# ipc-sim/IPC

Measured on AMD Instinct MI355X. Metric: newton_iterations_per_sec, higher is better.
Workload: dtype f64

## Files before the change

### ipc_amd/csrc/mf_numeric.hip

```cpp
#include <climits>
#include "mf_kernels.h"
#include "device_prims.h"
#include <algorithm>
#include <chrono>
#include <cstdio>
#include <cstdlib>
#include <cstring>
#include <thread>

namespace ipcgpu {

namespace {

__global__ void k_clear_flag(int* __restrict__ flag) { flag[0] = 0; }


struct EntryView {
    const int *ia, *ja;
    int nRows, ns;
    const int *newOf, *nodeFront, *firstNode, *idxPtr, *idx;
    const long long* frontOff;
    const int4* frontInfo;
};
__global__ __launch_bounds__(256) void k_entry_dst(EntryView v, long long* __restrict__ dst, int* __restrict__ bucket, int* __restrict__ hist)
{
    const int r = blockIdx.x * 4 + (threadIdx.x >> 6), lane = threadIdx.x & 63;
    if (r >= v.nRows) return;
    const int pr = 3 * v.newOf[r / 3] + r % 3;
    for (int k = v.ia[r] + lane; k < v.ia[r + 1]; k += 64) {
        const int c = v.ja[k];
        const int pc = 3 * v.newOf[c / 3] + c % 3;
        const int i = max(pr, pc), j = min(pr, pc);
        const int s = v.nodeFront[j / 3];
        const int f = v.firstNode[s], l = v.firstNode[s + 1];
        const int nIdx = v.idxPtr[s + 1] - v.idxPtr[s];
        int lr;
        if (i / 3 < l) lr = i - 3 * f;
        else {
            const int* b = v.idx + v.idxPtr[s] + (l - f);
            int lo = 0, hi = nIdx - (l - f);
            const int key = i / 3;
            while (lo < hi) {
                const int mid = (lo + hi) >> 1;
                if (b[mid] < key) lo = mid + 1;
                else hi = mid;
            }
            lr = 3 * ((l - f) + lo) + i % 3;
        }
        const int lc = j - 3 * f;
        dst[k] = v.frontOff[s] + lr + (long long)(3 * nIdx) * lc;
        const int4 info = v.frontInfo[s];
        int bkt = -1;
        if (info.x == 0) bkt = s;
        else if (info.x > 0) {
            const int ti = lr / TS, tj = lc / TS, cT = info.z;
            bkt = v.ns + info.y + (ti <= cT ? ti * (ti + 1) / 2 : cT * (cT + 1) / 2 + (ti - cT) * cT) + tj;
        }
        bucket[k] = bkt;
        if (bkt >= 0) atomicAdd(&hist[bkt], 1);
    }
}
__global__ __launch_bounds__(1024) void k_scan_exclusive(int n, const int* __restrict__ in, int* __restrict__ out)
{
    __shared__ int part[1024];
    const int t = threadIdx.x;
    const int chunk = (n + 1023) / 1024;
    const int b = min(t * chunk, n), e = min(b + chunk, n);
    int sum = 0;
    for (int i = b; i < e; ++i) sum += in[i];
    part[t] = sum;
    __syncthreads();
    for (int off = 1; off < 1024; off <<= 1) {
        const int x = (t >= off) ? part[t - off] : 0;
        __syncthreads();
        part[t] += x;
        __syncthreads();
    }
    int run = part[t] - sum;
    for (int i = b; i < e; ++i) {
        out[i] = run;
        run += in[i];
    }
    if (t == 1023) out[n] = part[1023];
}
__global__ void k_entry_scatter(int nnz, int ns, const long long* __restrict__ dst, const int* __restrict__ bucket, const int* __restrict__ start,
    int* __restrict__ cursor, const long long* __restrict__ frontOff, int2* __restrict__ aEnt, int* __restrict__ bigSrc,
    long long* __restrict__ bigDst)
{
    const int k = blockIdx.x * blockDim.x + threadIdx.x;
    if (k >= nnz) return;
    const int b = bucket[k];
    if (b < 0) return;
    const int pos = start[b] + atomicAdd(&cursor[b], 1);
    if (b < ns) {
        aEnt[pos] = make_int2((int)(dst[k] - frontOff[b]), k);
    }
    else {
        const int q = pos - start[ns];
        bigSrc[q] = k;
        bigDst[q] = dst[k];
    }
}

#ifdef MF_EA_PROBE
constexpr int EA_PROBE_PH = 8;
__device__ unsigned long long g_eaProbe[2][64][EA_PROBE_PH + 1];
struct EaProbe {
    unsigned long long t[EA_PROBE_PH];
};
#define EA_PROBE_DECL EaProbe pr_ = {}
#define EA_STAMP(k)                                                                                                                                           \
    do {                                                                                                                                                      \
        if (probeLevel >= 0) {                                                                                                                                \
            asm volatile("s_waitcnt vmcnt(0) lgkmcnt(0)" ::: "memory");                                                                                       \
            if (threadIdx.x == 0) pr_.t[k] = wall_clock64();                                                                                                  \
        }                                                                                                                                                     \
    } while (0)
__device__ inline void ea_probe_flush(const EaProbe& p, int kernel, int level)
{
    if (threadIdx.x != 0 || level < 0 || level >= 64) return;
    unsigned long long prev = p.t[0];
    for (int k = 1; k < EA_PROBE_PH; ++k) {
        const unsigned long long t = p.t[k] ? p.t[k] : prev;
        atomicAdd(&g_eaProbe[kernel][level][k], t - prev);
        prev = t;
    }
    atomicAdd(&g_eaProbe[kernel][level][EA_PROBE_PH], 1ull);
}
#define EA_PROBE_FLUSH(kernel) ea_probe_flush(pr_, kernel, probeLevel)
#else
#define EA_PROBE_DECL do {} while (0)
#define EA_STAMP(k) do {} while (0)
#define EA_PROBE_FLUSH(kernel) do {} while (0)
#endif

struct KidGather {
    double x[16];
    bool ok[16];
};
__device__ __forceinline__ void kid_gather(const double* __restrict__ Fc, const long long Nc, const int r, const int (&cc)[16], KidGather& g)
{
#pragma unroll
    for (int q = 0; q < 16; ++q) {
        g.ok[q] = r >= 0 && cc[q] >= 0 && r >= cc[q];
        g.x[q] = Fc[g.ok[q] ? r + Nc * cc[q] : 0];
    }
}
__device__ __forceinline__ const double* kid_front(const double* fronts, const int4 k)
{
    return fronts + (((long long)(unsigned)k.y << 32) | (unsigned)k.x);
}

__global__ __launch_bounds__(WG) void k_extend_add(const int4* __restrict__ tile, const int* __restrict__ childMap, const int4* __restrict__ kidRec,
    double* __restrict__ fronts, int ownOnly, const int* __restrict__ aPtr, const int* __restrict__ aSrc, const long long* __restrict__ aDst,
    const double* __restrict__ a
#ifdef MF_EA_PROBE
    ,
    int probeLevel
#endif
)
{
    EA_PROBE_DECL;
    EA_STAMP(0);
    const int4 g = tile[4 * blockIdx.x], t = tile[4 * blockIdx.x + 1], k0 = tile[4 * blockIdx.x + 2], k1 = tile[4 * blockIdx.x + 3];
    const int aBeg = aPtr[blockIdx.x], aEnd = aPtr[blockIdx.x + 1];
    const int tid = threadIdx.x, lane = tid & 63, wv = __builtin_amdgcn_readfirstlane(tid >> 6);
    const int e0 = aBeg + tid;
    long long dst0 = 0;
    double a0 = 0.0;
    if (e0 < aEnd) {
        dst0 = aDst[e0];
        a0 = a[aSrc[e0]];
    }
    EA_STAMP(1);
    const int N = g.x, ncOwn = g.y, nk = t.z;
    double* F = fronts + (((long long)(unsigned)g.w << 32) | (unsigned)g.z);
    const int I = TS * t.x + lane, J0 = TS * t.y + 16 * wv;
    const int* m0 = childMap + k0.w;
    const int* m1 = childMap + k1.w;
    const int r0 = m0[I], r1 = m1[I];
    int c0[16], c1[16];
#pragma unroll
    for (int q = 0; q < 16; ++q) {
        c0[q] = m0[J0 + q];
        c1[q] = m1[J0 + q];
    }
    EA_STAMP(2);
    KidGather g0, g1;
    kid_gather(kid_front(fronts, k0), k0.z, r0, c0, g0);
    kid_gather(kid_front(fronts, k1), k1.z, r1, c1, g1);
    double sum[16];
#pragma unroll
    for (int q = 0; q < 16; ++q) sum[q] = 0.0;
#pragma unroll
    for (int q = 0; q < 16; ++q) sum[q] += g0.ok[q] ? g0.x[q] : 0.0;
#pragma unroll
    for (int q = 0; q < 16; ++q) sum[q] += g1.ok[q] ? g1.x[q] : 0.0;
    EA_STAMP(4);
    for (int k = 2; k < nk; ++k) {
        const int4 kr = kidRec[t.w + k];
        const int* m = childMap + kr.w;
        const int r = m[I];
#pragma unroll
        for (int q = 0; q < 16; ++q) c0[q] = m[J0 + q];
        kid_gather(kid_front(fronts, kr), kr.z, r, c0, g0);
#pragma unroll
        for (int q = 0; q < 16; ++q) sum[q] += g0.ok[q] ? g0.x[q] : 0.0;
    }
    if (I < N) {
#pragma unroll
        for (int q = 0; q < 16; ++q) {
            const int J = J0 + q;
            if (J <= I && (!ownOnly || J < ncOwn)) F[I + (long long)N * J] = sum[q];
        }
    }
    EA_STAMP(6);
    if (aBeg < aEnd) {
        __syncthreads();
        if (e0 < aEnd) fronts[dst0] += a0;
        for (int e = e0 + WG; e < aEnd; e += WG) fronts[aDst[e]] += a[aSrc[e]];
    }
    EA_STAMP(7);
    EA_PROBE_FLUSH(0);
}

__device__ __forceinline__ double bcast_lane(double v, int lane)
{
    const int lo = __builtin_amdgcn_readlane(__double2loint(v), lane);
    const int hi = __builtin_amdgcn_readlane(__double2hiint(v), lane);
    return __hiloint2double(hi, lo);
}

__device__ __forceinline__ double rsqrt_nr(double d)
{
    double r = __builtin_amdgcn_rsq(d);
    double e = fma(-d * r, r, 1.0);
    r = fma(0.5 * r, e, r);
    e = fma(-d * r, r, 1.0);
    r = fma(0.5 * r, e, r);
    return r;
}

__device__ __forceinline__ double rcp_nr(double d)
{
    double r = __builtin_amdgcn_rcp(d);
    double e = fma(-d, r, 1.0);
    r = fma(r, e, r);
    e = fma(-d, r, 1.0);
    r = fma(r, e, r);
    return r;
}

__device__ __forceinline__ double lane_xor16(double v) { return __shfl_xor(v, 16, 64); }

__device__ __forceinline__ bool wave_potrf_inv32_mfma(const double* blk, int ld, int w, int lane, double* Xs)
{
    const int lo = lane & 15, hi = lane >> 4;
    f64x4 T00, T01, T11, W00, W11;
    f64x4 W10 = { 0.0, 0.0, 0.0, 0.0 };
    f64x4 aV0, bV0, dV0, alV0, cbV0, aV1, bV1, dV1;
    const int wm = w - 1;
#pragma unroll
    for (int r = 0; r < 4; ++r) {
        const int q = hi + 4 * r;
        const int mn = min(q, lo), mx = max(q, lo);
        const double a00 = blk[min(mn, wm) * ld + min(mx, wm)];
        const double a01 = blk[min(q, wm) * ld + min(16 + lo, wm)];
        const double a11 = blk[min(16 + mn, wm) * ld + min(16 + mx, wm)];
        const bool dg = q == lo;
        T00[r] = (mx < w) ? a00 : (dg ? 1.0 : 0.0);
        T01[r] = (16 + lo < w) ? a01 : 0.0;
        T11[r] = (16 + mx < w) ? a11 : (dg ? 1.0 : 0.0);
        W00[r] = dg ? 1.0 : 0.0;
        W11[r] = dg ? 1.0 : 0.0;
        aV0[r] = aV1[r] = dV0[r] = dV1[r] = 1.0;
        bV0[r] = bV1[r] = alV0[r] = cbV0[r] = 0.0;
    }
    bool bad = false;
#pragma unroll
    for (int k = 0; k < 16; k += 2) {
        if (k >= w) break;
        const int h = k & 3, r = k >> 2;
        const bool selh = hi == h, both = (hi >> 1) == (h >> 1), live = both && lo > k + 1;
        const double row = T00[r];
        const double partner = lane_xor16(row);
        const double a = bcast_lane(row, 16 * h + k), b = bcast_lane(row, 16 * h + k + 1), c = bcast_lane(row, 16 * (h + 1) + k + 1);
        const double det = fma(a, c, -(b * b));
        bad |= !(a > 0.0) || !(det > 0.0);
        const double rdet = rcp_nr(det);
        const double ca = c * rdet, cb = b * rdet, cc = a * rdet;
        const double alpha = selh ? ca : cc;
        const double m = live ? fma(-alpha, row, cb * partner) : 0.0;
        T00 = __builtin_amdgcn_mfma_f64_16x16x4f64(m, row, T00, 0, 0, 0);
        T01 = __builtin_amdgcn_mfma_f64_16x16x4f64(m, T01[r], T01, 0, 0, 0);
        W00 = __builtin_amdgcn_mfma_f64_16x16x4f64(m, W00[r], W00, 0, 0, 0);
        aV0[r] = both ? a : aV0[r];
        bV0[r] = both ? b : bV0[r];
        dV0[r] = both ? det : dV0[r];
        alV0[r] = both ? alpha : alV0[r];
        cbV0[r] = both ? cb : cbV0[r];
    }
    if (w > 16) {
#pragma unroll
        for (int ks = 0; ks < 4; ++ks) {
            const double t = T01[ks];
            const double a = fma(-alV0[ks], t, cbV0[ks] * lane_xor16(t));
            T11 = __builtin_amdgcn_mfma_f64_16x16x4f64(a, t, T11, 0, 0, 0);
            W10 = __builtin_amdgcn_mfma_f64_16x16x4f64(a, W00[ks], W10, 0, 0, 0);
        }
#pragma unroll
        for (int k = 0; k < 16; k += 2) {
            if (16 + k >= w) break;
            const int h = k & 3, r = k >> 2;
            const bool selh = hi == h, both = (hi >> 1) == (h >> 1), live = both && lo > k + 1;
            const double row = T11[r];
            const double partner = lane_xor16(row);
            const double a = bcast_lane(row, 16 * h + k), b = bcast_lane(row, 16 * h + k + 1), c = bcast_lane(row, 16 * (h + 1) + k + 1);
            const double det = fma(a, c, -(b * b));
            bad |= !(a > 0.0) || !(det > 0.0);
            const double rdet = rcp_nr(det);
            const double ca = c * rdet, cb = b * rdet, cc = a * rdet;
            const double alpha = selh ? ca : cc;
            const double m = live ? fma(-alpha, row, cb * partner) : 0.0;
            T11 = __builtin_amdgcn_mfma_f64_16x16x4f64(m, row, T11, 0, 0, 0);
            W11 = __builtin_amdgcn_mfma_f64_16x16x4f64(m, W11[r], W11, 0, 0, 0);
            aV1[r] = both ? a : aV1[r];
            bV1[r] = both ? b : bV1[r];
            dV1[r] = both ? det : dV1[r];
        }
    }
    const bool even = (hi & 1) == 0;
#pragma unroll
    for (int r = 0; r < 4; ++r) {
        const int q = hi + 4 * r;
        const double ia0 = rsqrt_nr(aV0[r]), iv0 = ia0 * ia0, il0 = rsqrt_nr(dV0[r] * iv0);
        const double ia1 = rsqrt_nr(aV1[r]), iv1 = ia1 * ia1, il1 = rsqrt_nr(dV1[r] * iv1);
        const double p0 = even ? ia0 : il0, q0 = even ? 0.0 : -bV0[r] * iv0 * il0;
        const double p1 = even ? ia1 : il1, q1 = even ? 0.0 : -bV1[r] * iv1 * il1;
        const double w0 = W00[r], w1 = W11[r];
        Xs[lo * LDX + q] = fma(q0, lane_xor16(w0), p0 * w0);
        Xs[(16 + lo) * LDX + 16 + q] = fma(q1, lane_xor16(w1), p1 * w1);
        Xs[(16 + lo) * LDX + q] = 0.0;
    }
    __builtin_amdgcn_fence(__ATOMIC_SEQ_CST, "wavefront");
    __builtin_amdgcn_wave_barrier();
    f64x4 X10 = { 0.0, 0.0, 0.0, 0.0 };
    if (w > 16) {
#pragma unroll
        for (int ks = 0; ks < 4; ++ks)
            X10 = __builtin_amdgcn_mfma_f64_16x16x4f64(Xs[(16 + 4 * ks + hi) * LDX + 16 + lo], W10[ks], X10, 0, 0, 0);
    }
#pragma unroll
    for (int r = 0; r < 4; ++r) Xs[lo * LDX + 16 + hi + 4 * r] = X10[r];
    __builtin_amdgcn_fence(__ATOMIC_SEQ_CST, "wavefront");
    __builtin_amdgcn_wave_barrier();
    return bad;
}

#ifndef MF_FUSED_SCHUR_GROUP
#define MF_FUSED_SCHUR_GROUP 2
#endif
#ifdef MF_FUSED_PROBE
__device__ unsigned long long g_probe[16 << 16];
__device__ const int* g_probeBase;
#define MF_PROBE(slot) do { if (tid == 0) g_probe[16 * probeId + (slot)] = wall_clock64(); } while (0)
#define MF_PROBE_ACC(var) do { if (tid == 0) { const unsigned long long now_ = wall_clock64(); var += now_ - probeLast; probeLast = now_; } } while (0)
#else
#define MF_PROBE(slot) do {} while (0)
#define MF_PROBE_ACC(var) do {} while (0)
#endif
template <int NT>
__global__ __launch_bounds__(NT, 3) void k_front_fused(const int* __restrict__ fdesc, const int* __restrict__ invMap,
    const int2* __restrict__ aEnt, const double* __restrict__ a, double* __restrict__ fronts,
    double* __restrict__ dinv, int* __restrict__ flag, int* __restrict__ flagNext)
{
    extern __shared__ double P[];
    __shared__ double Xs[NB * LDX];
    __shared__ __attribute__((aligned(16))) int fd[FD_STRIDE];
    const int tid = threadIdx.x, lane = tid & 63, wv = tid >> 6;
    if (tid < FD_STRIDE) fd[tid] = fdesc[(size_t)blockIdx.x * FD_STRIDE + tid];
    if (flagNext && blockIdx.x == 0 && tid == 0) flagNext[0] = 0;
    __syncthreads();
    const int N = fd[2], nc = fd[3], nk = fd[8];
    double* F = fronts + *reinterpret_cast<const long long*>(fd);
    double* dblk = dinv + *reinterpret_cast<const long long*>(fd + 4) * (NB * NB);
    const int aBeg = fd[6], aEnd = fd[7];
    int* cm = reinterpret_cast<int*>(P + (size_t)nc * N);
    bool bad = false;
#ifdef MF_FUSED_PROBE
    const long long probeId = ((fdesc - g_probeBase) / FD_STRIDE + blockIdx.x) & 0xffff;
    unsigned long long probeLast = 0, probePivot = 0, probeRows = 0, probeTrail = 0, probeGather = 0, probeTiles = 0;
    if (tid == 0) {
        g_probe[16 * probeId + 12] = N;
        g_probe[16 * probeId + 13] = nc;
        g_probe[16 * probeId + 14] = nk;
    }
#endif
    MF_PROBE(0);
    const int aLast = max(aEnd - 1, 0);
    int2 ent0[4];
    double av0[4];
#pragma unroll
    for (int u = 0; u < 4; ++u) ent0[u] = aEnt[min(aBeg + u * NT + tid, aLast)];
    for (int q = 0; q < nk; ++q) {
        const int* inv = invMap + fd[16 + 6 * q + 4];
        const int ncc = fd[16 + 6 * q + 3];
        for (int I = tid; I < N; I += NT) {
            const int In = I / 3;
            const int ic = inv[In];
            cm[q * N + I] = ic >= 0 ? ncc + 3 * ic + (I - 3 * In) : -1;
        }
    }
#pragma unroll
    for (int u = 0; u < 4; ++u) av0[u] = a[ent0[u].y];
    __syncthreads();
    MF_PROBE(1);
    for (int J0 = 2 * wv; J0 < nc; J0 += 2 * (NT / 64)) {
        const int Ja = J0, Jb = min(J0 + 1, nc - 1);
        for (int I0 = 0; I0 < N; I0 += 4 * 64) {
            double va[4] = { 0.0, 0.0, 0.0, 0.0 }, vb[4] = { 0.0, 0.0, 0.0, 0.0 };
#pragma unroll 2
            for (int q = 0; q < nk; ++q) {
                const double* Fc = fronts + *reinterpret_cast<const long long*>(fd + 16 + 6 * q);
                const long long Nc = fd[16 + 6 * q + 2];
                const int cca = cm[q * N + Ja], ccb = cm[q * N + Jb];
                double xa[4], xb[4];
                bool oka[4], okb[4];
#pragma unroll
                for (int u = 0; u < 4; ++u) {
                    const int I = I0 + 64 * u + lane;
                    const int r = (I < N) ? cm[q * N + I] : -1;
                    oka[u] = r >= 0 && cca >= 0 && I >= Ja;
                    okb[u] = r >= 0 && ccb >= 0 && I >= Jb;
                    xa[u] = Fc[oka[u] ? r + Nc * cca : 0];
                    xb[u] = Fc[okb[u] ? r + Nc * ccb : 0];
                }
#pragma unroll
                for (int u = 0; u < 4; ++u) {
                    va[u] += oka[u] ? xa[u] : 0.0;
                    vb[u] += okb[u] ? xb[u] : 0.0;
                }
            }
#pragma unroll
            for (int u = 0; u < 4; ++u) {
                const int I = I0 + 64 * u + lane;
                if (I < N) {
                    P[Ja * N + I] = va[u];
                    if (J0 + 1 < nc) P[Jb * N + I] = vb[u];
                }
            }
        }
    }
    __syncthreads();
    MF_PROBE(2);
#pragma unroll
    for (int u = 0; u < 4; ++u)
        if (aBeg + u * NT + tid < aEnd) P[ent0[u].x] += av0[u];
    for (int e0 = aBeg + 4 * NT; e0 < aEnd; e0 += 4 * NT) {
        int2 ent[4];
        double av[4];
#pragma unroll
        for (int u = 0; u < 4; ++u) ent[u] = aEnt[min(e0 + u * NT + tid, aLast)];
#pragma unroll
        for (int u = 0; u < 4; ++u) av[u] = a[ent[u].y];
#pragma unroll
        for (int u = 0; u < 4; ++u)
            if (e0 + u * NT + tid < aEnd) P[ent[u].x] += av[u];
    }
    __syncthreads();
    MF_PROBE(3);
#ifdef MF_FUSED_PROBE
    probeLast = wall_clock64();
#endif

    for (int kb = 0; kb < nc; kb += NB, dblk += NB * NB) {
        const int w = min(NB, nc - kb);
        double* Pk = P + (size_t)kb * N + kb;
        if (tid < 64) {
            __builtin_amdgcn_s_setprio(3);
            bad |= wave_potrf_inv32_mfma(Pk, N, w, tid, Xs);
            __builtin_amdgcn_s_setprio(0);
        }
        __syncthreads();
        MF_PROBE_ACC(probePivot);
        for (int e = tid; e < NB * NB; e += NT) dblk[e] = Xs[(e >> 5) * LDX + (e & 31)];
        {
            const int lo = lane & 15, hi = lane >> 4;
            const int R0 = kb + w, ntile = (N - R0 + 15) >> 4;
            for (int t = wv; t < ntile; t += NT / 64) {
                const int row = min(R0 + 16 * t + lo, N - 1);
                double bv[8];
#pragma unroll
                for (int ks = 0; ks < 8; ++ks) {
                    const int k = 4 * ks + hi;
                    const double v = P[(kb + min(k, w - 1)) * N + row];
                    bv[ks] = (k < w) ? v : 0.0;
                }
                f64x4 x0 = { 0.0, 0.0, 0.0, 0.0 }, x1 = { 0.0, 0.0, 0.0, 0.0 };
#pragma unroll
                for (int ks = 0; ks < 4; ++ks) x0 = __builtin_amdgcn_mfma_f64_16x16x4f64(Xs[(4 * ks + hi) * LDX + lo], bv[ks], x0, 0, 0, 0);
                if (w > 16) {
#pragma unroll
                    for (int ks = 0; ks < 8; ++ks)
                        x1 = __builtin_amdgcn_mfma_f64_16x16x4f64(Xs[(4 * ks + hi) * LDX + 16 + lo], bv[ks], x1, 0, 0, 0);
                }
                if (R0 + 16 * t + lo < N) {
#pragma unroll
                    for (int i = 0; i < 4; ++i) {
                        const int n0 = hi + 4 * i, n1 = 16 + hi + 4 * i;
                        if (n0 < w) P[(kb + n0) * N + row] = x0[i];
                        if (n1 < w) P[(kb + n1) * N + row] = x1[i];
                    }
                }
            }
        }
        __syncthreads();
        MF_PROBE_ACC(probeRows);
        const int c0 = kb + w;
        if (c0 < nc) {
            const int ntc = (nc - c0 + 3) >> 2, ntr = (N - c0 + 3) >> 2;
            for (int t = tid; t < ntc * ntr; t += NT) {
                const int tc = t / ntr, tr = t - tc * ntr;
                if (tr < tc) continue;
                const int i0 = c0 + 4 * tr, j0 = c0 + 4 * tc;
// ... 840 lines not shown
    };
    double va[2][4], vb[2][4], na[2][4], nb[2][4];
    int k0 = kBeg + 16 * wv;
    fetch(k0, va, vb);
    for (; k0 < kStop; k0 += 128) {
        fetch(k0 + 64, na, nb);
        __builtin_amdgcn_sched_barrier(0);
        mult(k0, va, vb);
        __builtin_amdgcn_sched_barrier(0);
        fetch(k0 + 128, va, vb);
        __builtin_amdgcn_sched_barrier(0);
        if (k0 + 64 < kStop) mult(k0 + 64, na, nb);
        __builtin_amdgcn_sched_barrier(0);
    }
#pragma unroll
    for (int a = 0; a < 2; ++a)
#pragma unroll
        for (int b = 0; b < 2; ++b)
#pragma unroll
            for (int i = 0; i < 4; ++i) red[wv][2 * a + b][64 * i + l] = acc[a][b][i];
    __syncthreads();
    const int a = wv >> 1, b = wv & 1;
    double* out = (mode == 1) ? T : X;
    const double sgn = (mode == 1) ? 1.0 : -1.0;
    const int r = r0 + 16 * b + lo;
#pragma unroll
    for (int i = 0; i < 4; ++i) {
        const int c = c0 + 16 * a + hi + 4 * i;
        const double v = ((red[0][wv][64 * i + l] + red[1][wv][64 * i + l]) + red[2][wv][64 * i + l]) + red[3][wv][64 * i + l];
        if (r < rEnd && c < cEnd) out[r + (long long)nc * c] = sgn * v;
    }
}

}

namespace {

static_assert(sizeof(MfRec4) == sizeof(int4) && alignof(MfRec4) <= alignof(int4), "the plan's records are uploaded as int4");
void uploadRecs(DevBuf<int4>& buf, const std::vector<MfRec4>& recs, hipStream_t stream) { buf.upload(reinterpret_cast<const int4*>(recs.data()), recs.size(), stream); }

}

void MfNumeric::setup(const MfSymbolic& sym, hipStream_t stream, const int* ia_dev, const int* ja_dev, long long nnzPattern)
{
    if (side_) HIP_CHECK(hipStreamSynchronize(side_));
    const bool timeIt = std::getenv("IPCGPU_MF_SETUP_TIMES") != nullptr;
    auto tSetup = std::chrono::steady_clock::now();
    auto lap = [&](const char* what) {
        if (!timeIt) return;
        HIP_CHECK(hipStreamSynchronize(stream));
        const auto now = std::chrono::steady_clock::now();
        fprintf(stderr, "mf setup %-28s %.2f ms\n", what, std::chrono::duration<double, std::milli>(now - tSetup).count());
        tSetup = now;
    };
    if (world_ > 64) throw StateError("the sharded solver supports at most 64 ranks");
    sym_ = &sym;
    stream_ = stream;
    ns_ = sym.ns;
    nLevels_ = (int)sym.levelPtr.size() - 1;
    fronts_.ensure((size_t)sym.frontOff[ns_]);
    fronts_.zeroN((size_t)sym.frontOff[ns_], stream);
    w_.alloc((size_t)sym.wOff[ns_]);
    yperm_.alloc((size_t)sym.n);
    bperm_.alloc((size_t)sym.n);
    xsol_.alloc((size_t)sym.n);
    idx_.upload(sym.idx, stream);
    idxPtr_.upload(sym.idxPtr, stream);
    firstNode_.upload(sym.firstNode, stream);
    childPtr_.upload(sym.childPtr, stream);
    child_.upload(sym.child.empty() ? std::vector<int>{ 0 } : sym.child, stream);
    invPtr_.upload(sym.invPtr, stream);
    inv_.upload(sym.inv.empty() ? std::vector<int>{ 0 } : sym.inv, stream);
    newOf_.upload(sym.newOf, stream);
    oldOf_.upload(sym.oldOf, stream);
    frontOff_.upload(std::vector<long long>(sym.frontOff.begin(), sym.frontOff.end()), stream);
    wOff_.upload(std::vector<long long>(sym.wOff.begin(), sym.wOff.end()), stream);
    lap("buffers + tree uploads");
    flag_.alloc(2);
    flag_.zero(stream);
    flagCur_ = 0;
    hflag_.alloc(4);
    auto newEvent = [] {
        hipEvent_t e;
        HIP_CHECK(hipEventCreateWithFlags(&e, hipEventDisableTiming));
        return e;
    };
    if (!side_) {
        HIP_CHECK(hipStreamCreateWithFlags(&side_, hipStreamNonBlocking));
        evSide_ = newEvent();
    }
    if (!fwd_) {
        HIP_CHECK(hipStreamCreateWithFlags(&fwd_, hipStreamNonBlocking));
        evRhs_ = newEvent();
        evFwdDone_ = newEvent();
    }
    while ((int)evFactLevel_.size() < nLevels_) evFactLevel_.push_back(newEvent());
    while ((int)evLevel_.size() < nLevels_) {
        evLevel_.push_back(newEvent());
        evInvDone_.push_back(newEvent());
    }
    sidePending_ = false;

    auto planning = [](auto&& step) {
        try {
            step();
        }
        catch (const MfPlanError& e) {
            throw StateError(e.what());
        }
    };
    mp_.rank = rank_;
    mp_.world = world_;
    mp_.tune = tune_;
    planning([&] { mf_plan_fronts(sym, mp_); });
    dinvOff_.upload(mp_.dinvOff, stream);
    dinv_.alloc((size_t)mp_.dinvOff[ns_] * NB * NB);
    const size_t nnz = (size_t)nnzPattern;
    const int nBuckets = ns_ + mp_.nEaTiles;
    uploadRecs(frontInfo_, mp_.frontInfo, stream);
    nodeFront_.upload(mp_.nodeFront, stream);
    entryDst_.ensure(nnz + 1);
    entryBucket_.ensure(nnz + 1);
    bucketHist_.ensure(2 * (size_t)nBuckets + 2);
    bucketStart_.ensure((size_t)nBuckets + 2);
    bucketHist_.zeroN(2 * (size_t)nBuckets + 2, stream);
    EntryView ev{ ia_dev, ja_dev, sym.n, ns_, newOf_.p, nodeFront_.p, firstNode_.p, idxPtr_.p, idx_.p, frontOff_.p, frontInfo_.p };
    hipLaunchKernelGGL(k_entry_dst, dim3((sym.n + 3) / 4), dim3(256), 0, stream, ev, entryDst_.p, entryBucket_.p, bucketHist_.p);
    hipLaunchKernelGGL(k_scan_exclusive, dim3(1), dim3(1024), 0, stream, nBuckets, bucketHist_.p, bucketStart_.p);
    std::vector<int> start((size_t)nBuckets + 1);
    bucketStart_.download(start.data(), start.size(), stream);
    const size_t nFused = (size_t)start[ns_], nBig = (size_t)(start[nBuckets] - start[ns_]);
    aEnt_.ensure(nFused + 1);
    aEnt_.zeroN(1, stream);
    bigASrc_.ensure(nBig + 1);
    bigADst_.ensure(nBig + 1);
    if (nnz)
        hipLaunchKernelGGL(k_entry_scatter, dim3((unsigned)((nnz + 255) / 256)), dim3(256), 0, stream, (int)nnz, ns_, entryDst_.p, entryBucket_.p, bucketStart_.p,
            bucketHist_.p + nBuckets + 1, frontOff_.p, aEnt_.p, bigASrc_.p, bigADst_.p);
    lap("A-entry lists");
    planning([&] { mf_plan_launches(sym, start.data(), mp_); });
    lap("level plans");
    eaAPtr_.upload(mp_.eaAPtr, stream);
    fdesc_.uploadGrow(mp_.fdesc, stream);
    lap("fused descriptors");
    triList_.upload(mp_.triList, stream);
    uploadRecs(xinvDesc_, mp_.xinvDesc, stream);
    xinvOff_.upload(mp_.xinvOff, stream);
    xinvX_.alloc((size_t)std::max<long long>(mp_.xTot, 1));
    xinvT_.alloc((size_t)std::max<long long>(mp_.xTot, 1));
    xinvX_.zero(stream);
    xinvT_.zero(stream);
    lap("inverse plan + buffers");
    smallList_.upload(mp_.smallList, stream);
    bigList_.upload(mp_.bigList, stream);
    childMap_.uploadGrow(mp_.childMap, stream);
    uploadRecs(kidRec_, mp_.kidRec, stream);
    eaTile_.uploadGrow(mp_.eaTile, stream);
    schurTile_.uploadGrow(mp_.schurTile, stream);
    uploadRecs(desc_, mp_.desc, stream);
    if (world_ > 1) {
        xchgBuf_.ensure((size_t)mp_.xchgStaging + 1);
        uploadRecs(xchgDesc_, mp_.xchgDesc, stream);
        nodeExec_.upload(mp_.nodeExec, stream);
        auto resolve = [](const std::vector<MfXchgOp>& ops, double* base, std::vector<P2POp>& out) {
            for (const MfXchgOp& o : ops) out.push_back(P2POp{ base + o.off, o.count, o.peer, o.send });
        };
        xchg_.assign(nLevels_, Xchg());
        for (int l = 0; l < nLevels_; ++l) {
            resolve(mp_.xchg[l].opsM, xchgBuf_.p, xchg_[l].opsM);
            resolve(mp_.xchg[l].opsW, xchgBuf_.p, xchg_[l].opsW);
            resolve(mp_.xchg[l].opsX, xsol_.p, xchg_[l].opsX);
        }
    }
    if (mp_.maxSmallLds > 48 * 1024) {
        HIP_CHECK(hipFuncSetAttribute((const void*)k_front_fused<256>, hipFuncAttributeMaxDynamicSharedMemorySize, (int)mp_.maxSmallLds));
        HIP_CHECK(hipFuncSetAttribute((const void*)k_front_fused<512>, hipFuncAttributeMaxDynamicSharedMemorySize, (int)mp_.maxSmallLds));
    }
    configureSweepKernels(mp_.maxSolveLds, mp_.maxBwdLds, mp_.maxTriLds);
    HIP_CHECK(hipStreamSynchronize(stream));
    lap("uploads + attributes");
}

void MfNumeric::nodeOwners(std::vector<int>& ownerOfNode) const
{
    if (!sym_) throw StateError("nodeOwners before analyze_pattern");
    const MfSymbolic& sym = *sym_;
    ownerOfNode.assign(sym.nn, -1);
    if (world_ <= 1) return;
    std::vector<int> perm(sym.nn, -1);
    for (int s = 0; s < ns_; ++s)
        for (int v = sym.firstNode[s]; v < sym.firstNode[s + 1]; ++v) perm[v] = mp_.owner[s];
    for (int v = 0; v < sym.nn; ++v) ownerOfNode[v] = perm[sym.newOf[v]];
}

MfNumeric::~MfNumeric()
{
    if (side_) (void)hipStreamSynchronize(side_);
    if (fwd_) (void)hipStreamSynchronize(fwd_);
    for (hipEvent_t e : evFactLevel_) (void)hipEventDestroy(e);
    if (evRhs_) (void)hipEventDestroy(evRhs_);
    if (evFwdDone_) (void)hipEventDestroy(evFwdDone_);
    if (fwd_) (void)hipStreamDestroy(fwd_);
    for (hipEvent_t e : evLevel_) (void)hipEventDestroy(e);
    for (hipEvent_t e : evInvDone_) (void)hipEventDestroy(e);
    if (evSide_) (void)hipEventDestroy(evSide_);
    if (side_) (void)hipStreamDestroy(side_);
}

bool MfNumeric::factorize(const double* a_dev)
{
    if (!sym_) throw StateError("factorize before analyze_pattern");
    enqueueFactor(a_dev);
    if (world_ > 1) {
        allreduceFlag();
    }
    prims::launch_publish(curFlag(), hflag_.dev, 1, stream_);
    HIP_CHECK(hipStreamSynchronize(stream_));
#ifdef MF_FUSED_PROBE
    {
        static int calls = 0;
        if (++calls == 3) {
            std::vector<unsigned long long> h(16 << 16);
            HIP_CHECK(hipMemcpyFromSymbol(h.data(), HIP_SYMBOL(g_probe), h.size() * sizeof(unsigned long long)));
            const char* names[7] = { "maps", "children", "A", "panels", "store", "schur", "total" };
            for (int l = 0; l < nLevels_; ++l) {
                const LevelPlan& P = mp_.level[l];
                if (!P.small.cnt) continue;
                double sum[16] = { 0 }, mx = 0;
                for (int b = 0; b < P.small.cnt; ++b) {
                    const unsigned long long* r = h.data() + 16 * (size_t)((P.small.off + b) & 0xffff);
                    for (int k = 0; k < 6; ++k) sum[k] += (double)(r[k + 1] - r[k]);
                    sum[6] += (double)(r[6] - r[0]);
                    mx = std::max(mx, (double)(r[6] - r[0]));
                    for (int k = 8; k < 16; ++k) sum[k] += (double)r[k];
                }
                const double c = 0.01 / P.small.cnt;
                std::fprintf(stderr, "[fused probe] level %d: %d fronts, %d threads, N %.0f nc %.0f kids %.1f |", l, P.small.cnt, P.smallThreads, sum[12] / P.small.cnt, sum[13] / P.small.cnt,
                    sum[14] / P.small.cnt);
                for (int k = 0; k < 7; ++k) std::fprintf(stderr, " %s %.2f", names[k], sum[k] * c);
                std::fprintf(stderr, " us (max %.2f) | inside panels: pivot %.2f rows %.2f trailing %.2f | inside schur (wave 0): gathers %.2f products + stores %.2f\n", mx * 0.01, sum[8] * c, sum[9] * c,
                    sum[10] * c, sum[11] * c, sum[15] * c);
            }
        }
    }
#endif
    return pivotsOk();
}

bool MfNumeric::pivotsOk() const
{
    return hflag_.p[0] == 0;
}

bool MfNumeric::factorizeSolve(const double* a_dev, const double* rhs_dev, double* x_dev, bool wait, bool negateRhs)
{
    if (!sym_) throw StateError("factorize before analyze_pattern");
    if (world_ > 1 || !fwd_) {
        const bool ok = factorize(a_dev);
        if (ok) solve(rhs_dev, x_dev, negateRhs);
        return ok;
    }
    HIP_CHECK(hipEventRecord(evRhs_, stream_));
    HIP_CHECK(hipStreamWaitEvent(fwd_, evRhs_, 0));
    enqueuePermuteRhs(rhs_dev, fwd_, negateRhs);
    fwdJoined_ = false;
    enqueueFactor(a_dev, true);
    if (!fwdJoined_) HIP_CHECK(hipEventRecord(evFwdDone_, fwd_));
    if (!fwdJoined_) HIP_CHECK(hipStreamWaitEvent(stream_, evFwdDone_, 0));
    enqueueBackward(x_dev, true);
    if (!wait) return true;
    HIP_CHECK(hipStreamSynchronize(stream_));
    return pivotsOk();
}

void MfNumeric::enqueueFactor(const double* a_dev, bool overlapForward)
{
    TreeView tv{ frontOff_.p, idxPtr_.p, firstNode_.p, childPtr_.p, child_.p, invPtr_.p, inv_.p, idx_.p, dinvOff_.p };
    XinvView xvF{ xinvOff_.p, xinvX_.p, xinvT_.p };
    if (sidePending_) HIP_CHECK(hipStreamWaitEvent(stream_, evSide_, 0));
    bool sideUsed = false;
    int fwdNext = 0;
#ifdef MF_FUSED_PROBE
    {
        const int* base = fdesc_.p;
        HIP_CHECK(hipMemcpyToSymbolAsync(HIP_SYMBOL(g_probeBase), &base, sizeof(base), 0, hipMemcpyHostToDevice, stream_));
    }
#endif
#ifdef MF_EA_PROBE
    static int eaProbeCalls = 0;
    const bool probeCall = ++eaProbeCalls == 20;
    if (eaProbeCalls == 21) {
        HIP_CHECK(hipStreamSynchronize(stream_));
        static unsigned long long h[2][64][EA_PROBE_PH + 1];
        HIP_CHECK(hipMemcpyFromSymbol(h, HIP_SYMBOL(g_eaProbe), sizeof(h)));
        const char* kn[2] = { "k_extend_add", "k_big_schur64_ea" };
        const char* names[EA_PROBE_PH] = { "", "records", "maps", "child0", "children", "product", "store", "A" };
        for (int k = 0; k < 2; ++k)
            for (int l = 0; l < nLevels_ && l < 64; ++l) {
                const double n = (double)h[k][l][EA_PROBE_PH];
                if (n == 0) continue;
                double tot = 0;
                std::fprintf(stderr, "[ea probe] %-16s level %2d: %5.0f workgroups |", kn[k], l, n);
                for (int ph = 1; ph < EA_PROBE_PH; ++ph) {
                    std::fprintf(stderr, " %s %.2f", names[ph], 0.01 * (double)h[k][l][ph] / n);
                    tot += 0.01 * (double)h[k][l][ph] / n;
                }
                std::fprintf(stderr, " | total %.2f us\n", tot);
            }
    }
#endif
    flagCur_ ^= 1;
    int* const flag = flag_.p + flagCur_;
    int* flagNext = flag_.p + (flagCur_ ^ 1);
    for (int l = 0; l < nLevels_; ++l) {
        const LevelPlan& P = mp_.level[l];
        if (P.small.cnt)
        {
            const int* fd = fdesc_.p + (size_t)P.small.off * FD_STRIDE;
            if (P.smallThreads == 512)
                hipLaunchKernelGGL(k_front_fused<512>, dim3(P.small.cnt), dim3(512), P.smallLds, stream_, fd, inv_.p, aEnt_.p, a_dev, fronts_.p,
                    dinv_.p, flag, flagNext);
            else
                hipLaunchKernelGGL(k_front_fused<256>, dim3(P.small.cnt), dim3(256), P.smallLds, stream_, fd, inv_.p, aEnt_.p, a_dev, fronts_.p,
                    dinv_.p, flag, flagNext);
            flagNext = nullptr;
        }
        if (P.ea.cnt) {
            const int4* tiles = reinterpret_cast<const int4*>(eaTile_.p + (size_t)P.ea.off * TILE_REC);
#ifdef MF_EA_PROBE
            hipLaunchKernelGGL(k_extend_add, dim3(P.ea.cnt), dim3(WG), 0, stream_, tiles, childMap_.p, kidRec_.p, fronts_.p, P.fuseEA ? 1 : 0, eaAPtr_.p + P.ea.off,
                bigASrc_.p, bigADst_.p, a_dev, probeCall ? l : -1);
#else
            hipLaunchKernelGGL(k_extend_add, dim3(P.ea.cnt), dim3(WG), 0, stream_, tiles, childMap_.p, kidRec_.p, fronts_.p, P.fuseEA ? 1 : 0, eaAPtr_.p + P.ea.off,
                bigASrc_.p, bigADst_.p, a_dev);
#endif
        }
        for (const Range& R : P.step) {
            if (!R.cnt) continue;
            if (P.stepTop) hipLaunchKernelGGL(k_big_step<true>, dim3(R.cnt), dim3(WGB), 0, stream_, desc_.p + R.off, tv, fronts_.p, dinv_.p, flag, xvF);
            else hipLaunchKernelGGL(k_big_step<false>, dim3(R.cnt), dim3(WGB), 0, stream_, desc_.p + R.off, tv, fronts_.p, dinv_.p, flag, xvF);
            const Range& U = P.bulk[&R - P.step.data()];
            if (U.cnt) hipLaunchKernelGGL(k_big_bulk, dim3(U.cnt), dim3(WG), 0, stream_, desc_.p + U.off, fronts_.p);
        }
        if (P.schur.cnt) {
            if (P.fuseEA) {
                const int4* tiles = reinterpret_cast<const int4*>(schurTile_.p + (size_t)P.schurTileOff * TILE_REC);
#ifdef MF_EA_PROBE
                hipLaunchKernelGGL(k_big_schur64_ea, dim3(P.schur.cnt), dim3(WG), 0, stream_, tiles, childMap_.p, kidRec_.p, fronts_.p, probeCall ? l : -1);
#else
                hipLaunchKernelGGL(k_big_schur64_ea, dim3(P.schur.cnt), dim3(WG), 0, stream_, tiles, childMap_.p, kidRec_.p, fronts_.p);
#endif
            }
            else if (P.schur64) hipLaunchKernelGGL(k_big_schur64, dim3(P.schur.cnt), dim3(WG), 0, stream_, desc_.p + P.schur.off, fronts_.p);
            else hipLaunchKernelGGL(k_big_schur, dim3(P.schur.cnt), dim3(WG), 0, stream_, desc_.p + P.schur.off, fronts_.p);
        }
        if (world_ > 1) exchangeUpdateMatrices(l);
        if (mp_.xinvLevel[l].blocks.cnt) {
            if (side_) {
                HIP_CHECK(hipEventRecord(evLevel_[l], stream_));
                HIP_CHECK(hipStreamWaitEvent(side_, evLevel_[l], 0));
                enqueueInverses(l, side_);
                HIP_CHECK(hipEventRecord(evInvDone_[l], side_));
                sideUsed = true;
            }
            else enqueueInverses(l, stream_);
        }
        if (overlapForward) {
            if (l == nLevels_ - 1 && !sideUsed) {
                HIP_CHECK(hipEventRecord(evFwdDone_, fwd_));
                HIP_CHECK(hipStreamWaitEvent(stream_, evFwdDone_, 0));
                enqueueForwardLevel(l, stream_);
                fwdJoined_ = true;
            }
            else if (l >= nLevels_ - 2 || (l + 1) % fwdStride_ == 0) {
                HIP_CHECK(hipEventRecord(evFactLevel_[l], stream_));
                HIP_CHECK(hipStreamWaitEvent(fwd_, evFactLevel_[l], 0));
                for (; fwdNext <= l; ++fwdNext) {
                    if (mp_.level[fwdNext].xinvFwd.cnt && sideUsed) HIP_CHECK(hipStreamWaitEvent(fwd_, evInvDone_[fwdNext], 0));
                    enqueueForwardLevel(fwdNext, fwd_);
                }
            }
        }
    }
    if (sideUsed) HIP_CHECK(hipEventRecord(evSide_, side_));
    sidePending_ = sideUsed;
    if (flagNext) hipLaunchKernelGGL(k_clear_flag, dim3(1), dim3(1), 0, stream_, flagNext);
}

void MfNumeric::enqueueInverses(int l, hipStream_t st)
{
    const XinvLevel& XL = mp_.xinvLevel[l];
    TreeView tv{ frontOff_.p, idxPtr_.p, firstNode_.p, childPtr_.p, child_.p, invPtr_.p, inv_.p, idx_.p, dinvOff_.p };
    XinvView xv{ xinvOff_.p, xinvX_.p, xinvT_.p };
    hipLaunchKernelGGL(k_xinv_init, dim3(XL.init.cnt), dim3(256), 0, st, xinvDesc_.p + XL.init.off, tv, xv, dinv_.p);
    for (const auto& R : XL.rounds) {
        if (R.first.cnt) hipLaunchKernelGGL(k_xinv_gemm, dim3(R.first.cnt), dim3(256), 0, st, xinvDesc_.p + 2 * (size_t)R.first.off, tv, xv, fronts_.p);
        if (R.second.cnt) hipLaunchKernelGGL(k_xinv_gemm, dim3(R.second.cnt), dim3(256), 0, st, xinvDesc_.p + 2 * (size_t)R.second.off, tv, xv, fronts_.p);
    }
}

}
```

Measured before the change: 458.7.

## Scatter original-matrix entries into LDS tile and fold into extend-add sum

Instead of scattering original matrix entries into the front with read-modify-write global stores after the extend-add writes, each workgroup zeroes a shared tile, scatters its entries into it by computing the tile-local slot, and adds the tile into the register sums before the single store. Entry index loads are prefetched for two rounds and issued early to overlap with child gathers. This removes a trailing global RMW pass and a barrier-ordered dependency on the front, at the cost of LDS usage, extra barriers and a float-based division for slot computation.

Result: no change. 461.8, median of 6 (+0.7%).

```diff
diff --git a/ipc_amd/csrc/mf_numeric.hip b/ipc_amd/csrc/mf_numeric.hip
--- a/ipc_amd/csrc/mf_numeric.hip
+++ b/ipc_amd/csrc/mf_numeric.hip
@@ -151,6 +151,23 @@
     return fronts + (((long long)(unsigned)k.y << 32) | (unsigned)k.x);
 }
 
+__device__ __forceinline__ int ea_tile_slot(int rel, int N, float rN)
+{
+    int c = (int)((float)rel * rN);
+    int r = rel - c * N;
+    if (r < 0) {
+        --c;
+        r += N;
+    }
+    else if (r >= N) {
+        ++c;
+        r -= N;
+    }
+    return r + TS * c;
+}
+
+constexpr int EA_R = 2;
+
 __global__ __launch_bounds__(WG) void k_extend_add(const int4* __restrict__ tile, const int* __restrict__ childMap, const int4* __restrict__ kidRec,
     double* __restrict__ fronts, int ownOnly, const int* __restrict__ aPtr, const int* __restrict__ aSrc, const long long* __restrict__ aDst,
     const double* __restrict__ a
@@ -160,21 +177,26 @@
 #endif
 )
 {
+    __shared__ double2 aT[TS * TS / 2];
     EA_PROBE_DECL;
     EA_STAMP(0);
     const int4 g = tile[4 * blockIdx.x], t = tile[4 * blockIdx.x + 1], k0 = tile[4 * blockIdx.x + 2], k1 = tile[4 * blockIdx.x + 3];
     const int aBeg = aPtr[blockIdx.x], aEnd = aPtr[blockIdx.x + 1];
     const int tid = threadIdx.x, lane = tid & 63, wv = __builtin_amdgcn_readfirstlane(tid >> 6);
+    const bool hasA = aBeg < aEnd;
     const int e0 = aBeg + tid;
-    long long dst0 = 0;
-    double a0 = 0.0;
-    if (e0 < aEnd) {
-        dst0 = aDst[e0];
-        a0 = a[aSrc[e0]];
-    }
-    EA_STAMP(1);
+    long long dstR[EA_R];
+    int srcR[EA_R];
+    double aR[EA_R];
+#pragma unroll
+    for (int r = 0; r < EA_R; ++r) {
+        const int e = e0 + r * WG < aEnd ? e0 + r * WG : 0;
+        dstR[r] = aDst[e];
+        srcR[r] = aSrc[e];
+    }
     const int N = g.x, ncOwn = g.y, nk = t.z;
-    double* F = fronts + (((long long)(unsigned)g.w << 32) | (unsigned)g.z);
+    const long long fOff = ((long long)(unsigned)g.w << 32) | (unsigned)g.z;
+    double* F = fronts + fOff;
     const int I = TS * t.x + lane, J0 = TS * t.y + 16 * wv;
     const int* m0 = childMap + k0.w;
     const int* m1 = childMap + k1.w;
@@ -185,10 +207,30 @@
         c0[q] = m0[J0 + q];
         c1[q] = m1[J0 + q];
     }
-    EA_STAMP(2);
+    if (hasA) {
+#pragma unroll
+        for (int k = 0; k < TS * TS / 2 / WG; ++k) aT[tid + WG * k] = make_double2(0.0, 0.0);
+    }
+#pragma unroll
+    for (int r = 0; r < EA_R; ++r)
+        aR[r] = a[e0 + r * WG < aEnd ? srcR[r] : 0];
+    EA_STAMP(1);
     KidGather g0, g1;
     kid_gather(kid_front(fronts, k0), k0.z, r0, c0, g0);
     kid_gather(kid_front(fronts, k1), k1.z, r1, c1, g1);
+    EA_STAMP(4);
+    if (hasA) {
+        double* const aS = reinterpret_cast<double*>(aT);
+        const long long tile0 = fOff + TS * t.x + (long long)N * (TS * t.y);
+        const float rN = 1.0f / (float)N;
+        __syncthreads();
+#pragma unroll
+        for (int r = 0; r < EA_R; ++r)
+            if (e0 + r * WG < aEnd) aS[ea_tile_slot((int)(dstR[r] - tile0), N, rN)] = aR[r];
+        for (int e = e0 + EA_R * WG; e < aEnd; e += WG) aS[ea_tile_slot((int)(aDst[e] - tile0), N, rN)] = a[aSrc[e]];
+        __syncthreads();
+    }
+    EA_STAMP(5);
     double sum[16];
 #pragma unroll
     for (int q = 0; q < 16; ++q) sum[q] = 0.0;
@@ -196,7 +238,6 @@
     for (int q = 0; q < 16; ++q) sum[q] += g0.ok[q] ? g0.x[q] : 0.0;
 #pragma unroll
     for (int q = 0; q < 16; ++q) sum[q] += g1.ok[q] ? g1.x[q] : 0.0;
-    EA_STAMP(4);
     for (int k = 2; k < nk; ++k) {
         const int4 kr = kidRec[t.w + k];
         const int* m = childMap + kr.w;
@@ -207,6 +248,11 @@
 #pragma unroll
         for (int q = 0; q < 16; ++q) sum[q] += g0.ok[q] ? g0.x[q] : 0.0;
     }
+    if (hasA) {
+        const double* const aS = reinterpret_cast<const double*>(aT);
+#pragma unroll
+        for (int q = 0; q < 16; ++q) sum[q] += aS[lane + TS * (16 * wv + q)];
+    }
     if (I < N) {
 #pragma unroll
         for (int q = 0; q < 16; ++q) {
@@ -215,11 +261,6 @@
         }
     }
     EA_STAMP(6);
-    if (aBeg < aEnd) {
-        __syncthreads();
-        if (e0 < aEnd) fronts[dst0] += a0;
-        for (int e = e0 + WG; e < aEnd; e += WG) fronts[aDst[e]] += a[aSrc[e]];
-    }
     EA_STAMP(7);
     EA_PROBE_FLUSH(0);
 }
@@ -1666,7 +1707,7 @@
                 double tot = 0;
                 std::fprintf(stderr, "[ea probe] %-16s level %2d: %5.0f workgroups |", kn[k], l, n);
                 for (int ph = 1; ph < EA_PROBE_PH; ++ph) {
-                    std::fprintf(stderr, " %s %.2f", names[ph], 0.01 * (double)h[k][l][ph] / n);
+                    std::fprintf(stderr, " %s %.2f", k == 0 && ph == 5 ? "entries" : names[ph], 0.01 * (double)h[k][l][ph] / n);
                     tot += 0.01 * (double)h[k][l][ph] / n;
                 }
                 std::fprintf(stderr, " | total %.2f us\n", tot);
```
